# CliffKai/BridgeLang

Measured on AMD Instinct MI355X. Metric: action-seqs/sec (7-DoF, 224px) openvla-7b bf16, higher is better.
Workload: dtype bf16; 1 GPU; openvla-7b bf16 inference (BASELINE configs[1]): batch 16 synthetic 224px frames + 32-token prompts per GPU, predict_action = vision towers + projector + Llama prefill S=288 + 6 cached decode steps, greedy; 7 batches in flight: per step one batch is submitted (vision+prefill) while decode iteration g of the batch submitted g steps earlier, g = 1..6, runs as ONE merged 96-row pass over the weights ; batch_per_gpu=16, prompt_len=32, seq_len=288, replicas=1, hip_graph=True, pipeline_depth=7

## Files before the change

bridgelang_amd/_lib.py:

```python
from __future__ import annotations

import ctypes as C
import os
from pathlib import Path

_HERE = Path(__file__).resolve().parent
LIB_PATH = _HERE / "libbridgelang_hip.so"

BL_OK, BL_E_SHAPE, BL_E_ALIGN, BL_E_LAUNCH, BL_E_ARG = 0, -1, -2, -3, -4
_ERR = {BL_E_SHAPE: "BL_E_SHAPE (unsupported shape)", BL_E_ALIGN: "BL_E_ALIGN (alignment)",
        BL_E_LAUNCH: "BL_E_LAUNCH (HIP launch failed)", BL_E_ARG: "BL_E_ARG (null pointer / bad enum)"}

EPI_NONE, EPI_BIAS, EPI_BIAS_GELU, EPI_BIAS_RES, EPI_RES, EPI_SWIGLU, EPI_F32, EPI_F32_BF16R = range(8)
EPI_SWIGLU_KEEP, EPI_BIAS_GELU_KEEP, EPI_SWIGLU_BWD, EPI_GELU_BWD = range(8, 12)


class GemmDesc(C.Structure):
    _fields_ = [
        ("A", C.c_void_p), ("lda", C.c_int64),
        ("W", C.c_void_p), ("ldw", C.c_int64),
        ("C", C.c_void_p), ("ldc", C.c_int64),
        ("M", C.c_int32), ("N", C.c_int32), ("K", C.c_int32),
        ("epilogue", C.c_int32),
        ("bias", C.c_void_p),
# ... 14 lines not shown
    _fields_ = [("kind", C.c_int32), ("nblocks", C.c_int32), ("rows", C.c_int32), ("cols", C.c_int32), ("rows_pad", C.c_int32),
                ("bx_count", C.c_int32), ("ld", C.c_int64), ("kt_total", C.c_int64), ("kb_off", C.c_int64), ("n", C.c_int64),
                ("src", C.c_void_p), ("dst", C.c_void_p), ("scale", C.c_float), ("pad", C.c_int32)]


class AttnDesc(C.Structure):
    _fields_ = [
        ("q", C.c_void_p), ("q_bs", C.c_int64), ("q_hs", C.c_int64), ("q_rs", C.c_int64),
        ("k", C.c_void_p), ("k_bs", C.c_int64), ("k_hs", C.c_int64), ("k_rs", C.c_int64),
        ("v", C.c_void_p), ("v_bs", C.c_int64), ("v_hs", C.c_int64), ("v_rs", C.c_int64),
        ("o", C.c_void_p), ("o_bs", C.c_int64), ("o_hs", C.c_int64), ("o_rs", C.c_int64),
        ("key_mask", C.c_void_p), ("mask_bs", C.c_int64),
        ("B", C.c_int32), ("H", C.c_int32), ("Sq", C.c_int32), ("Skv", C.c_int32), ("head_dim", C.c_int32),
        ("causal", C.c_int32),
        ("scale", C.c_float),
    ]


_vp, _i32, _i64, _u32, _f32 = C.c_void_p, C.c_int32, C.c_int64, C.c_uint32, C.c_float

SIGNATURES = {
    "bl_abi_version": (C.c_int, []),
    "bl_build_arch": (C.c_char_p, []),
    "bl_fill_synth_bf16": (C.c_int, [_vp, _i64, _u32, _f32, _f32, _vp]),
    "bl_fill_synth_bf16_2d": (C.c_int, [_vp, _i64, _i64, _i64, _u32, _f32, _f32, _vp]),
    "bl_pack_weight_bf16": (C.c_int, [_vp, _i64, _i64, _i64, _vp, _vp]),
    "bl_gemm_fp8": (C.c_int, [C.POINTER(GemmDesc), _vp, _vp, _vp]),
    "bl_quantize_rows_fp8": (C.c_int, [_vp, _i64, _i32, _i32, _vp, _i64, _vp, _vp]),
    "bl_colamax_bf16": (C.c_int, [_vp, _i64, _i32, _i32, _vp, _vp]),
    "bl_transpose_quantize_fp8": (C.c_int, [_vp, _i64, _i32, _i32, _vp, _vp, _i64, _i32, _vp, _vp]),
    "bl_gemm_bf16": (C.c_int, [C.POINTER(GemmDesc), _vp]),
    "bl_gemm_skinny_bf16": (C.c_int, [C.POINTER(GemmDesc), _vp]),
    "bl_gemm_skinny_rows_bf16": (C.c_int, [C.POINTER(GemmDesc), _vp]),
    "bl_gemm_tn_bf16": (C.c_int, [C.POINTER(GemmDesc), _vp]),
    "bl_rmsnorm_skinny_bf16": (C.c_int, [_vp, _i64, _vp, _vp, _i64, _i32, _i32, _f32, _vp]),
    "bl_layernorm_bf16": (C.c_int, [_vp, _i64, _vp, _vp, _vp, _i64, _i32, _i32, _f32, _vp]),
    "bl_rmsnorm_bf16": (C.c_int, [_vp, _i64, _vp, _vp, _i64, _i32, _i32, _f32, _vp]),
    "bl_attention_bf16": (C.c_int, [C.POINTER(AttnDesc), _vp]),
    "bl_attention_rope_bf16": (C.c_int, [C.POINTER(AttnDesc), _vp, _vp, _i32, _vp, _vp, _i32, _vp]),
    "bl_attention_lse_bf16": (C.c_int, [C.POINTER(AttnDesc), _vp, _vp]),
    "bl_attention_backward_bf16": (C.c_int, [C.POINTER(AttnDesc), _vp, _vp, _vp, _vp, _vp, _vp, _vp]),
    "bl_attention_decode_bf16": (C.c_int, [C.POINTER(AttnDesc), _vp]),
    "bl_attention_decode_rope_bf16": (C.c_int, [C.POINTER(AttnDesc), _vp, _vp, _i32, _vp]),
    "bl_attention_decode_rope_pos_bf16": (C.c_int, [C.POINTER(AttnDesc), _vp, _vp, _i32, _vp, _vp]),
    "bl_attention_decode_rope_grouped_bf16": (C.c_int, [C.POINTER(AttnDesc), _vp, _vp, _i32, _vp, _vp, _vp, _vp]),
    "bl_rope_kvcache_bf16": (C.c_int, [_vp, _i32, _i32, _i32, _i32, _vp, _vp, _i32, _vp, _vp, _i32, _vp]),
    "bl_embed_splice_bf16": (C.c_int, [_vp, _i32, _i32, _vp, _i32, _i32, _vp, _vp]),
    "bl_argmax_f32": (C.c_int, [_vp, _i64, _i32, _i32, _vp, _vp]),
    "bl_cross_entropy_f32": (C.c_int, [_vp, _i64, _i32, _i32, _vp, _i64, _vp, _vp, _vp]),
    "bl_cross_entropy_backward_f32": (C.c_int, [_vp, _i64, _i32, _i32, _vp, _i64, _vp, _vp, _i64, _vp]),
    "bl_rmsnorm_backward_bf16": (C.c_int, [_vp, _i64, _vp, _vp, _i64, _vp, _i64, _vp, _i64, _vp, _vp, _i64, _i32, _i32, _f32, _vp]),
    "bl_layernorm_backward_bf16": (C.c_int, [_vp, _i64, _vp, _vp, _i64, _vp, _i64, _vp, _i64, _vp, _vp, _vp, _i64, _i32, _i32, _f32, _vp]),
    "bl_colsum_bf16": (C.c_int, [_vp, _i64, _i32, _i32, _vp, _vp, _i64, _vp]),
    "bl_swiglu_bf16": (C.c_int, [_vp, _i64, _vp, _i64, _i64, _i32, _vp]),
    "bl_swiglu_backward_bf16": (C.c_int, [_vp, _i64, _vp, _i64, _vp, _i64, _i64, _i32, _vp]),
    "bl_gelu_bf16": (C.c_int, [_vp, _i64, _vp, _i64, _i64, _i32, _vp]),
    "bl_gelu_backward_bf16": (C.c_int, [_vp, _i64, _vp, _i64, _vp, _i64, _i64, _i32, _vp]),
    "bl_rope_backward_bf16": (C.c_int, [_vp, _i64, _i32, _i32, _i32, _i32, _vp, _vp, _i32, _vp]),
    "bl_transpose_pad_bf16": (C.c_int, [_vp, _i64, _i32, _i32, _vp, _i64, _i32, _vp]),
    "bl_pack_weight_into_bf16": (C.c_int, [_vp, _i64, _i64, _i64, _vp, _i64, _i64, _vp]),
    "bl_transpose_pack_into_bf16": (C.c_int, [_vp, _i64, _i32, _i32, _vp, _i32, _i64, _i64, _vp]),
    "bl_transpose_pack_bf16": (C.c_int, [_vp, _i64, _i32, _i32, _vp, _i32, _vp]),
    "bl_sumsq_partial_f32": (C.c_int, [_vp, _i64, _vp, _i32, _vp]),
    "bl_clip_coef_f32": (C.c_int, [_vp, _i32, _f32, _vp, _vp]),
    "bl_adamw_f32": (C.c_int, [_vp, _vp, _vp, _vp, _vp, _i64, _f32, _f32, _f32, _f32, _f32, _i32, _vp, _vp]),
    "bl_rope_bf16": (C.c_int, [_vp, _i64, _i32, _i32, _i32, _i32, _vp, _vp, _i32, _vp]),
# ... 51 lines not shown
```

bridgelang_amd/csrc/gemm_bf16.hip:

```cpp
#include "gemm_common.h"
#include <stdlib.h>

namespace bl_gemm_bf16_impl {
using namespace blgemm;

constexpr int BK = 64;
constexpr int ROW_BYTES = 128;
constexpr int GROUP_M = 4;

__device__ __forceinline__ void lin_to_tile(const GemmArgs& p, int lin, int& tm, int& tn) {
  const int width = GROUP_M * p.tiles_n, grp = lin / width, first = grp * GROUP_M;
  const int gsz = min(p.tiles_m - first, GROUP_M), rem = lin - grp * width;
  tm = first + rem % gsz;
  tn = rem / gsz;
}

__device__ __forceinline__ void tile_coords(const GemmArgs& p, int& tm, int& tn) {
  const int nwg = gridDim.x;
  const int orig = blockIdx.x, xcd = orig & 7, q = nwg >> 3, r = nwg & 7;
  const int lin = (xcd < r ? xcd * (q + 1) : r * (q + 1) + (xcd - r) * q) + (orig >> 3);
  const int width = GROUP_M * p.tiles_n, grp = lin / width, first = grp * GROUP_M;
  const int gsz = min(p.tiles_m - first, GROUP_M), rem = lin - grp * width;
  tm = first + rem % gsz;
  tn = rem / gsz;
// ... 1121 lines not shown
  f32x4_t sum = {0.f, 0.f, 0.f, 0.f};
  for (int s = 0; s < p.splitk; ++s)
    sum += *(const f32x4_t*)(p.slab + (((long)(tile_local * p.splitk + s) * 32 + idx) * 512 + tid) * 4);
  epilogue_store4<EPI>(p, tm * 256 + wm * 128 + j * 16 + l15,
                       TN ? tn * 256 + (i >> 1) * 128 + wn * 32 + (i & 1) * 16 + lg * 4 : tn * 256 + wn * 64 + i * 16 + lg * 4, sum);
}

constexpr int CUS = 256;
constexpr int LDS128 = 2 * 256 * ROW_BYTES, LDS256 = 2 * 65536, LDS288 = 2 * 73728;
constexpr int ring8_lds_bytes(int bm, int bn) { return 4 * (bm + bn) * ROW_BYTES + 1024; }

template <typename Kernel>
bool lds_attr(Kernel* kernel, int bytes) {
  return hipFuncSetAttribute(reinterpret_cast<const void*>(kernel), hipFuncAttributeMaxDynamicSharedMemorySize, bytes) ==
         hipSuccess;
}

template <int MB, int NB>
constexpr int mid_lds_bytes() { return 3 * (64 * MB * ROW_BYTES + NB * 2048); }
template <int EPI, int MB, int NB, int SK = 0>
bool mid_attr() { return lds_attr(&gemm_mid_kernel<EPI, MB, NB, SK>, mid_lds_bytes<MB, NB>()); }

constexpr int RS_LDS_BYTES = 4 * 2 * 6 * 16 * ROW_BYTES;
template <int EPI, int NWV, int SK>
int launch_rs(const GemmArgs& p, hipStream_t s, int n_tiles) {
  static const int attr_rc = lds_attr(&gemm_rows_stream_kernel<EPI, NWV, SK>, RS_LDS_BYTES) ? BL_OK : BL_E_LAUNCH;
  if (attr_rc != BL_OK) return attr_rc;
  hipLaunchKernelGGL((gemm_rows_stream_kernel<EPI, NWV, SK>), dim3((n_tiles + NWV - 1) / NWV, 8 / SK), dim3(NWV * 64),
                     RS_LDS_BYTES, s, p, n_tiles);
  return BL_OK;
}

template <int EPI>
int launch_rows_sk(const GemmArgs& a, hipStream_t s) {
  static const int attr_rc = mid_attr<EPI, 2, 4, 8>() && mid_attr<EPI, 2, 4, 2>() ? BL_OK : BL_E_LAUNCH;
  if (attr_rc != BL_OK) return attr_rc;
  GemmArgs p = a;
  p.fold_ks = p.K / 256;
  const int n_tiles = p.N / 16;
  const char* e_on = getenv("BL_ROWS_STREAM");
  if (p.M <= 96 && p.fold_ks % 4 == 0 && n_tiles > 256 && (e_on ? atoi(e_on) : 1)) {
    const bool can_split = p.slab && p.slab_bytes >= 2L * p.M * p.N * 4;
    int rc;
    if ((n_tiles + 7) / 8 >= 200) {
      p.splitk = 1;
      rc = launch_rs<EPI, 8, 8>(p, s, n_tiles);
    } else if ((n_tiles + 5) / 6 >= 200 || !can_split) {
      p.splitk = 1;
      rc = launch_rs<EPI, 6, 8>(p, s, n_tiles);
    } else {
      p.splitk = 2;
      rc = launch_rs<BL_EPI_NONE, 8, 4>(p, s, n_tiles);
      const long work = (long)p.M * (p.N / 4);
      if (rc == BL_OK)
        hipLaunchKernelGGL((gemm_rows_tree_reduce_kernel<EPI>), dim3((int)min((work + 255) / 256, 2048L)), dim3(256), 0, s, p);
    }
    if (rc != BL_OK) return rc;
    BL_CHECK_LAUNCH();
    return BL_OK;
  }
  const int slabs64 = (p.N + 63) / 64;
  const bool split = slabs64 * 2 <= 256 && p.slab && p.slab_bytes >= 4L * p.M * p.N * 4;
  p.splitk = split ? 4 : 1;
  if (split) {
    hipLaunchKernelGGL((gemm_mid_kernel<EPI, 2, 4, 2>), dim3(slabs64, 4), dim3(256), (mid_lds_bytes<2, 4>()), s, p);
    const long work = (long)p.M * (p.N / 4);
    hipLaunchKernelGGL((gemm_rows_tree_reduce_kernel<EPI>), dim3((int)min((work + 255) / 256, 2048L)), dim3(256), 0, s, p);
  } else {
    hipLaunchKernelGGL((gemm_mid_kernel<EPI, 2, 4, 8>), dim3(slabs64), dim3(256), (mid_lds_bytes<2, 4>()), s, p);
  }
  BL_CHECK_LAUNCH();
  return BL_OK;
}

template <int EPI>
int set_lds_attr() {
  static const int rc = [] {
    const bool ok =
        lds_attr(&gemm256s_kernel<EPI>, LDS256) && lds_attr(&gemm288s_kernel<EPI>, LDS288) &&
        lds_attr(&gemm128_kernel<EPI>, LDS128) &&
        lds_attr(&gemm_ring8_kernel<EPI, 160, 128, 4>, ring8_lds_bytes(160, 128)) &&
        lds_attr(&gemm_ring8_kernel<EPI, 128, 128, 4>, ring8_lds_bytes(128, 128)) &&
        lds_attr(&gemm_ring8_kernel<EPI, 128, 64, 4>, ring8_lds_bytes(128, 64)) &&
        lds_attr(&gemm_ring8_kernel<EPI, 64, 64, 4>, ring8_lds_bytes(64, 64)) &&
        lds_attr(&gemm_mid2_kernel<EPI, 1>, 3 * (160 * ROW_BYTES + 4096)) &&
        lds_attr(&gemm_mid2_kernel<EPI, 4>, 3 * (160 * ROW_BYTES + 4 * 4096)) &&
        lds_attr(&gemm_mid2_kernel<EPI, 2, 2>, 2 * (160 * ROW_BYTES + 2 * 4096)) &&
        mid_attr<EPI, 2, 4>() && mid_attr<EPI, 4, 4>() && mid_attr<EPI, 5, 4>() && mid_attr<EPI, 2, 1>() &&
        mid_attr<EPI, 4, 1>() && mid_attr<EPI, 5, 1>();
    return ok ? BL_OK : BL_E_LAUNCH;
  }();
  return rc;
}

template <int EPI>
void launch_slab_reduce(const GemmArgs& p, hipStream_t s) {
  const long work = (long)p.M * (p.N / 4);
  hipLaunchKernelGGL((gemm128_splitk_reduce_kernel<EPI>), dim3((int)min((work + 255) / 256, 2048L)), dim3(256), 0, s, p);
}

template <int EPI, int MB>
void launch_mid(const GemmArgs& p, hipStream_t s, bool wide, dim3 grid) {
  if (wide) hipLaunchKernelGGL((gemm_mid_kernel<EPI, MB, 4>), grid, dim3(256), (mid_lds_bytes<MB, 4>()), s, p);
  else hipLaunchKernelGGL((gemm_mid_kernel<EPI, MB, 1>), grid, dim3(256), (mid_lds_bytes<MB, 1>()), s, p);
}
// ... 175 lines not shown
    case BL_EPI_NONE: return launch_gemm<BL_EPI_NONE>(a, s);
    case BL_EPI_BIAS: return launch_gemm<BL_EPI_BIAS>(a, s);
    case BL_EPI_BIAS_GELU: return launch_gemm<BL_EPI_BIAS_GELU>(a, s);
    case BL_EPI_BIAS_RES: return launch_gemm<BL_EPI_BIAS_RES>(a, s);
    case BL_EPI_RES: return launch_gemm<BL_EPI_RES>(a, s);
    case BL_EPI_SWIGLU: return launch_gemm<BL_EPI_SWIGLU>(a, s);
    case BL_EPI_F32: return launch_gemm<BL_EPI_F32>(a, s);
    case BL_EPI_F32_BF16R: return launch_gemm<BL_EPI_F32_BF16R>(a, s);
    case BL_EPI_SWIGLU_KEEP: return launch_gemm<BL_EPI_SWIGLU_KEEP>(a, s);
    case BL_EPI_BIAS_GELU_KEEP: return launch_gemm<BL_EPI_BIAS_GELU_KEEP>(a, s);
    case BL_EPI_SWIGLU_BWD: return launch_gemm<BL_EPI_SWIGLU_BWD>(a, s);
    case BL_EPI_GELU_BWD: return launch_gemm<BL_EPI_GELU_BWD>(a, s);
    default: return BL_E_ARG;
  }
}

extern "C" int bl_gemm_skinny_rows_bf16(const bl_gemm_desc* d, void* stream) {
  GemmArgs a;
  const int rc = fill_gemm_args(d, a);
  if (rc != BL_OK) return rc;
  if (d->M > 128 || (d->K % 256) || d->a_norm_weight) return BL_E_SHAPE;
  if (d->out_group) return BL_E_ARG;
  hipStream_t s = (hipStream_t)stream;
  switch (d->epilogue) {
    case BL_EPI_NONE: return launch_rows_sk<BL_EPI_NONE>(a, s);
    case BL_EPI_RES: return launch_rows_sk<BL_EPI_RES>(a, s);
    case BL_EPI_SWIGLU: return launch_rows_sk<BL_EPI_SWIGLU>(a, s);
    case BL_EPI_F32: return launch_rows_sk<BL_EPI_F32>(a, s);
    case BL_EPI_F32_BF16R: return launch_rows_sk<BL_EPI_F32_BF16R>(a, s);
    default: return BL_E_ARG;
  }
}

extern "C" int bl_gemm_tn_bf16(const bl_gemm_desc* d, void* stream) {
  if (!d || !d->A || !d->W || !d->C) return BL_E_ARG;
  if (d->epilogue != BL_EPI_F32 || d->out_group || d->a_norm_weight) return BL_E_ARG;
  if (d->M <= 0 || d->N <= 0 || d->K <= 0 || (d->M % 8) || (d->N % 8)) return BL_E_SHAPE;
  if ((d->lda % 8) || (d->ldw % 8) || (d->ldc % 4) || d->lda < d->M || d->ldw < d->N || d->ldc < d->N) return BL_E_ALIGN;
  if (!bl_aligned16(d->A) || !bl_aligned16(d->W) || (((uintptr_t)d->C) & 15)) return BL_E_ALIGN;
  if ((long)d->K * d->lda * 2 >= (1L << 31) || (long)d->K * d->ldw * 2 >= (1L << 31)) return BL_E_SHAPE;
  GemmArgs a = {};
  a.A = d->A; a.W = d->W; a.C = d->C;
  a.lda = d->lda; a.ldw = d->ldw; a.ldc = d->ldc;
  a.M = d->M; a.N = d->N; a.K = d->K;
  a.tail_base = -1;
  a.slab = (float*)d->workspace; a.slab_bytes = d->workspace_bytes; a.splitk = 1;
  return launch_gemm_tn(a, (hipStream_t)stream);
}
```

bridgelang_amd/csrc/gemm_common.h:

```cpp
#pragma once
#include "bl_common.h"

namespace blgemm {

struct GemmArgs {
  const uint16_t* A; const uint16_t* W; void* C;
  const uint16_t* bias; const uint16_t* scale; const uint16_t* res;
  long lda, ldw, ldc, ldres;
  int M, N, K;
  int res_row_mod, out_group, out_stride, out_offset;
  int tiles_m, tiles_n;
  const uint16_t* norm_w; float norm_eps;
  float* slab; long slab_bytes; int splitk;
  int tail_base;
  const float* qa; const float* qw;
  int fold_ks;
  uint16_t* C2; long ldc2;
  int ptiles;
};

__device__ __forceinline__ int out_row_of(const GemmArgs& p, int m) {
  if (p.out_group == 0) return m;
  const int g = m / p.out_group, r = m - g * p.out_group + p.out_offset;
  if (r < 0 || r >= p.out_stride) return -1;
  return g * p.out_stride + r;
}

template <int EPI>
__device__ __forceinline__ void epilogue_store4(const GemmArgs& p, int m, int n, f32x4_t acc) {
  if (m >= p.M || n >= p.N) return;
  const int orow = out_row_of(p, m);
  if (orow < 0) return;
  if constexpr (EPI == BL_EPI_F32 || EPI == BL_EPI_F32_BF16R) {
    float* c = (float*)p.C + (long)orow * p.ldc + n;
    if constexpr (EPI == BL_EPI_F32_BF16R) acc = (f32x4_t){rbf(acc[0]), rbf(acc[1]), rbf(acc[2]), rbf(acc[3])};
    *(f32x4_t*)c = acc;
    return;
  } else if constexpr (EPI == BL_EPI_SWIGLU_KEEP) {
    const float g0 = rbf(acc[0]), u0 = rbf(acc[1]), g1 = rbf(acc[2]), u1 = rbf(acc[3]);
    u32x2_t o; o[0] = pack2bf(g0, u0); o[1] = pack2bf(g1, u1);
    *(u32x2_t*)((uint16_t*)p.C + (long)orow * p.ldc + n) = o;
    *(uint32_t*)(p.C2 + (long)orow * p.ldc2 + (n >> 1)) = pack2bf(rbf(silu_f(g0)) * u0, rbf(silu_f(g1)) * u1);
    return;
  } else if constexpr (EPI == BL_EPI_SWIGLU_BWD) {
    float v[8], o[8];
    const u32x4_t q = *(const u32x4_t*)(p.res + (long)m * p.ldres + 2 * n);
#pragma unroll
    for (int i = 0; i < 4; ++i) { v[2 * i] = bflo(q[i]); v[2 * i + 1] = bfhi(q[i]); }
#pragma unroll
    for (int e = 0; e < 4; ++e) swiglu_bwd_pair(v[2 * e], v[2 * e + 1], rbf(acc[e]), o[2 * e], o[2 * e + 1]);
    u32x4_t w;
#pragma unroll
// ... 227 lines not shown
```

bridgelang_amd/csrc/gemm_skinny.hip:

```cpp
#include "gemm_common.h"

namespace bl_gemm_skinny_impl {
using namespace blgemm;

constexpr int NW = 8;

template <int KS>
__device__ __forceinline__ void load_x_fragments(const uint16_t* A, long lda, int M, int l15, long kbase,
                                                 bf16x8_t (&xf)[KS]) {
  const bool live = l15 < M;
  const uint16_t* xp = A + (long)(live ? l15 : M - 1) * lda + kbase;
#pragma unroll
  for (int s = 0; s < KS; ++s) {
    u32x4_t t = *(const u32x4_t*)(xp + s * 32);
    if (!live) t = (u32x4_t){0u, 0u, 0u, 0u};
    xf[s] = __builtin_bit_cast(bf16x8_t, t);
  }
}

template <int KS>
__device__ __forceinline__ void rmsnorm_fragments(const uint16_t* norm_w, float eps, int K, long kbase, int wave, int l15,
                                                  int lg, float (&nrm)[8][16], bf16x8_t (&xf)[KS]) {
  u32x4_t gw[KS];
  {
// ... 88 lines not shown
                          ((r[4][lane] + r[5][lane]) + (r[6][lane] + r[7][lane]));
      epilogue_store4<EPI>(p, l15, tile * 16 + lg * 4, sum);
    }
  }
#undef BL_LOAD_GROUP
}

template <int KS, int GS, int EPI>
int launch_ks(const GemmArgs& a, hipStream_t s) {
  const int n_tiles = a.N / 16;
  const int tpw = (n_tiles + 255) / 256;
  const int grid = (n_tiles + tpw - 1) / tpw;
  if (a.norm_w) hipLaunchKernelGGL((gemm_skinny_kernel<KS, GS, EPI, true>), dim3(grid), dim3(NW * 64), 0, s, a, n_tiles);
  else hipLaunchKernelGGL((gemm_skinny_kernel<KS, GS, EPI, false>), dim3(grid), dim3(NW * 64), 0, s, a, n_tiles);
  BL_CHECK_LAUNCH();
  return BL_OK;
}

template <int EPI>
int launch_skinny(const GemmArgs& a, hipStream_t s) {
  switch (a.K) {
    case 4096: return launch_ks<16, 8, EPI>(a, s);
    case 11008: return launch_ks<43, 8, EPI>(a, s);
    case 5120: return launch_ks<20, 5, EPI>(a, s);
    case 13824: return launch_ks<54, 9, EPI>(a, s);
    case 512: return launch_ks<2, 1, EPI>(a, s);
    case 1024: return launch_ks<4, 2, EPI>(a, s);
    case 1536: return launch_ks<6, 3, EPI>(a, s);
    default: return BL_E_SHAPE;
  }
}


template <int KS>
__global__ __launch_bounds__(NW * 64) void rmsnorm_skinny_kernel(const uint16_t* x, long ldx, const uint16_t* w,
                                                                 uint16_t* y, long ldy, int rows, int K, float eps) {
  __shared__ float nrm[NW][16];
  const int tid = threadIdx.x, lane = tid & 63, wave = tid >> 6;
  const int l15 = lane & 15, lg = lane >> 4;
  const long kbase = (long)wave * (KS * 32) + lg * 8;
  const int row0 = blockIdx.x * 16, m = min(16, rows - row0);
  bf16x8_t xf[KS];
  load_x_fragments<KS>(x + (long)row0 * ldx, ldx, m, l15, kbase, xf);
  rmsnorm_fragments<KS>(w, eps, K, kbase, wave, l15, lg, nrm, xf);
  if (l15 < m) {
    uint16_t* yp = y + (long)(row0 + l15) * ldy + kbase;
#pragma unroll
    for (int s = 0; s < KS; ++s) *(u32x4_t*)(yp + s * 32) = __builtin_bit_cast(u32x4_t, xf[s]);
  }
}

template <int KS>
int launch_norm_skinny(const uint16_t* x, long ldx, const uint16_t* w, uint16_t* y, long ldy, int rows, int K, float eps,
                       hipStream_t s) {
  hipLaunchKernelGGL((rmsnorm_skinny_kernel<KS>), dim3((rows + 15) / 16), dim3(NW * 64), 0, s, x, ldx, w, y, ldy, rows, K, eps);
  BL_CHECK_LAUNCH();
  return BL_OK;
}

}
using namespace bl_gemm_skinny_impl;

extern "C" int bl_gemm_skinny_bf16(const bl_gemm_desc* d, void* stream) {
  GemmArgs a;
  const int rc = fill_gemm_args(d, a);
  if (rc != BL_OK) return rc;
  if (d->M > 16) return BL_E_SHAPE;
  hipStream_t s = (hipStream_t)stream;
  switch (d->epilogue) {
    case BL_EPI_NONE: return launch_skinny<BL_EPI_NONE>(a, s);
    case BL_EPI_RES: return launch_skinny<BL_EPI_RES>(a, s);
    case BL_EPI_SWIGLU: return launch_skinny<BL_EPI_SWIGLU>(a, s);
    case BL_EPI_F32: return launch_skinny<BL_EPI_F32>(a, s);
    case BL_EPI_F32_BF16R: return launch_skinny<BL_EPI_F32_BF16R>(a, s);
    default: return BL_E_ARG;
  }
}

extern "C" int bl_rmsnorm_skinny_bf16(const bl_bf16* x, int64_t ldx, const bl_bf16* w, bl_bf16* y, int64_t ldy,
                                      int32_t rows, int32_t dim, float eps, void* stream) {
  if (!x || !w || !y) return BL_E_ARG;
  if (rows <= 0) return BL_E_SHAPE;
  if ((ldx % 8) || (ldy % 8) || ldx < dim || ldy < dim || !bl_aligned16(x) || !bl_aligned16(y) || !bl_aligned16(w))
    return BL_E_ALIGN;
  hipStream_t s = (hipStream_t)stream;
  switch (dim) {
    case 4096: return launch_norm_skinny<16>(x, ldx, w, y, ldy, rows, dim, eps, s);
    case 11008: return launch_norm_skinny<43>(x, ldx, w, y, ldy, rows, dim, eps, s);
    case 5120: return launch_norm_skinny<20>(x, ldx, w, y, ldy, rows, dim, eps, s);
    case 13824: return launch_norm_skinny<54>(x, ldx, w, y, ldy, rows, dim, eps, s);
    case 512: return launch_norm_skinny<2>(x, ldx, w, y, ldy, rows, dim, eps, s);
    case 1024: return launch_norm_skinny<4>(x, ldx, w, y, ldy, rows, dim, eps, s);
    case 1536: return launch_norm_skinny<6>(x, ldx, w, y, ldy, rows, dim, eps, s);
    default: return BL_E_SHAPE;
// ... 3 lines not shown
```

bridgelang_amd/ops.py:

```python
from __future__ import annotations

import functools
import math

import ctypes as C
from typing import Optional, Sequence, Tuple

import torch

from . import _lib
from ._lib import (AttnDesc, GemmDesc, EPI_BIAS, EPI_BIAS_GELU, EPI_BIAS_GELU_KEEP, EPI_BIAS_RES, EPI_F32, EPI_F32_BF16R, EPI_GELU_BWD,
                   EPI_NONE, EPI_SWIGLU_BWD, EPI_SWIGLU_KEEP,
                   EPI_RES, EPI_SWIGLU)

__all__ = ["Op", "gemm", "gemm_fp8", "quantize_rows_fp8", "quantize_weight_fp8", "pack_weight", "unpack_weight", "cross_entropy", "layernorm", "rmsnorm", "rmsnorm_skinny", "skinny_rows_supported", "attention", "attention_rope", "attention_decode", "attention_decode_rope", "attention_decode_rope_grouped", "skinny_supported", "rope_kvcache", "embed_splice",
           "argmax", "im2col_patch14", "preprocess_u8", "resample_coeffs", "resize_bicubic_u8", "resize_u8", "crop_resize_bilinear_u8", "write_prefix_tokens", "fill_synth", "run_all",
           "EPI_NONE", "EPI_BIAS", "EPI_BIAS_GELU", "EPI_BIAS_RES", "EPI_RES", "EPI_SWIGLU", "EPI_F32", "EPI_F32_BF16R",
           "EPI_SWIGLU_KEEP", "EPI_BIAS_GELU_KEEP", "EPI_SWIGLU_BWD", "EPI_GELU_BWD"]


def _stream() -> int:
    return torch.cuda.current_stream().cuda_stream


# ... 42 lines not shown
    lib = _lib.load()
    _bf16(w, "w")
    N, K = w.shape
    if out is None:
        out = torch.empty(N // 16, K // 32, 64, 8, dtype=torch.bfloat16, device=w.device)
    _lib.check(lib.bl_pack_weight_bf16(w.data_ptr(), _rows(w, "w"), N, K, _bf16(out, "out").data_ptr(), _stream()),
               "bl_pack_weight_bf16")
    return out


def unpack_weight(wp: torch.Tensor) -> torch.Tensor:
    nt, ks = wp.shape[0], wp.shape[1]
    return wp.view(nt, ks, 4, 16, 8).permute(0, 3, 1, 2, 4).reshape(nt * 16, ks * 32)


SKINNY_K = (512, 1024, 1536, 4096, 5120, 11008, 13824)
_SKINNY_EPI = (EPI_NONE, EPI_RES, EPI_SWIGLU, EPI_F32, EPI_F32_BF16R)


def skinny_supported(M: int, K: int, epilogue: int) -> bool:
    return M <= 16 and K in SKINNY_K and epilogue in _SKINNY_EPI


def skinny_rows_supported(M: int, K: int, epilogue: int) -> bool:
    return M <= 128 and K in SKINNY_K and epilogue in _SKINNY_EPI


def gemm(A: torch.Tensor, W: torch.Tensor, out: torch.Tensor, epilogue: int = EPI_NONE, *,
         bias: Optional[torch.Tensor] = None, scale: Optional[torch.Tensor] = None,
         res: Optional[torch.Tensor] = None, res_row_mod: int = 0,
         out_map: Optional[Tuple[int, int, int]] = None,
         skinny: Optional[bool] = None, algo_nk: Optional[Tuple[int, int]] = None,
         a_norm: Optional[Tuple[torch.Tensor, float]] = None, workspace: Optional[torch.Tensor] = None,
         skinny_rows: bool = False, out2: Optional[torch.Tensor] = None, run: bool = True) -> Op:
    lib = _lib.load()
    _bf16(A, "A"); _bf16(W, "W")
    if W.dim() != 4 or W.shape[2:] != (64, 8) or not W.is_contiguous():
        raise ValueError(f"gemm: W must be a packed weight [N/16, K/32, 64, 8] (ops.pack_weight), got {tuple(W.shape)}")
    M, K = A.shape
    N, Kw = W.shape[0] * 16, W.shape[1] * 32
    if Kw != K:
        raise ValueError(f"gemm: K mismatch A{tuple(A.shape)} W(packed) K={Kw}")
    want = torch.float32 if epilogue in (EPI_F32, EPI_F32_BF16R) else torch.bfloat16
    if out.dtype != want or not out.is_cuda:
        raise TypeError(f"gemm: out must be {want} on device")
    d = GemmDesc()
    d.A, d.lda = A.data_ptr(), _rows(A, "A")
    d.W, d.ldw = W.data_ptr(), K
    d.C, d.ldc = out.data_ptr(), _rows(out, "out")
    d.M, d.N, d.K, d.epilogue = M, N, K, epilogue
    keep = [A, W, out]
    if bias is not None:
        d.bias = _bf16(bias, "bias").data_ptr(); keep.append(bias)
    if scale is not None:
        d.scale = _bf16(scale, "scale").data_ptr(); keep.append(scale)
    if res is not None:
        d.res, d.ldres = _bf16(res, "res").data_ptr(), _rows(res, "res"); keep.append(res)
    d.res_row_mod = res_row_mod
    if epilogue in (EPI_SWIGLU_KEEP, EPI_BIAS_GELU_KEEP):
        if out2 is None:
            raise ValueError("gemm: the *_KEEP epilogues need out2")
        n2 = N // 2 if epilogue == EPI_SWIGLU_KEEP else N
        if out2.shape[1] < n2 or out2.shape[0] < M:
            raise ValueError(f"gemm: out2 {tuple(out2.shape)} too small for [{M}, {n2}]")
        d.C2, d.ldc2 = _bf16(out2, "out2").data_ptr(), _rows(out2, "out2"); keep.append(out2)
    elif out2 is not None:
        raise ValueError("gemm: out2 only with the *_KEEP epilogues")
    if epilogue in (EPI_SWIGLU_BWD, EPI_GELU_BWD) and (res is None or res.shape[0] < M or
                                                       res.shape[1] < (2 * N if epilogue == EPI_SWIGLU_BWD else N)):
        raise ValueError("gemm: the *_BWD epilogues read the saved pre-activation through res")
    if out_map is not None:
        d.out_group, d.out_stride, d.out_offset = out_map
    if workspace is not None:
        d.workspace, d.workspace_bytes = workspace.data_ptr(), workspace.numel() * workspace.element_size()
        keep.append(workspace)
    n_out = N // 2 if epilogue == EPI_SWIGLU else 2 * N if epilogue == EPI_SWIGLU_BWD else N
    if out.shape[1] < n_out:
        raise ValueError(f"gemm: out has {out.shape[1]} columns, needs {n_out}")
    if out_map is None and out.shape[0] < M:
        raise ValueError(f"gemm: out has {out.shape[0]} rows, needs {M}")
    use_skinny = skinny
    if use_skinny is None:
        use_skinny = skinny_supported(M, K, epilogue)
    if a_norm is not None:
        if not use_skinny:
            raise ValueError("gemm: a_norm (fused RMSNorm) needs the skinny kernel (M <= 16 and a supported K)")
        d.a_norm_weight, d.a_norm_eps = _bf16(a_norm[0], "a_norm weight").data_ptr(), float(a_norm[1])
        keep.append(a_norm[0])
    if skinny_rows:
        if not skinny_rows_supported(M, K, epilogue) or a_norm is not None or out_map is not None:
            raise ValueError(f"gemm: skinny_rows needs M <= 128, K in {SKINNY_K}, no a_norm / out_map (M={M}, K={K})")
        name = "bl_gemm_skinny_rows_bf16"
    else:
        name = "bl_gemm_skinny_bf16" if use_skinny else "bl_gemm_bf16"
    fn = getattr(lib, name)
    esz = 4 if epilogue in (EPI_F32, EPI_F32_BF16R) else 2
    op = Op(name, fn, (C.byref(d),), (d, *keep),
            flops=2.0 * M * (algo_nk[0] if algo_nk else N) * (algo_nk[1] if algo_nk else K),
            nbytes=2.0 * (M * K + N * K) + esz * M * n_out)
    if run:
        op.run()
    return op


FP8_MAX = 448.0


def quantize_weight_fp8(w: torch.Tensor) -> Tuple[torch.Tensor, torch.Tensor]:
    N, K = w.shape
    if N % 16 or K % 128:
        raise ValueError("quantize_weight_fp8: N % 16 == 0 and K % 128 == 0")
    wf = w.float()
    amax = wf.abs().amax(dim=1)
    scale = torch.where(amax > 0, amax / FP8_MAX, torch.ones_like(amax))
    q = (wf / scale[:, None]).to(torch.float8_e4m3fn)
    packed = pack_weight(q.view(torch.uint8).view(N, K // 2, 2).view(torch.bfloat16).reshape(N, K // 2).contiguous())
    return packed, scale.contiguous()


def quantize_rows_fp8(x: torch.Tensor, q: Optional[torch.Tensor] = None, scales: Optional[torch.Tensor] = None,
                      run: bool = True):
    lib = _lib.load()
    _bf16(x, "x")
    rows, cols = x.shape
    if q is None:
        q = torch.empty(rows, cols, dtype=torch.uint8, device=x.device)
    if scales is None:
        scales = torch.empty(rows, dtype=torch.float32, device=x.device)
    op = Op("bl_quantize_rows_fp8", lib.bl_quantize_rows_fp8,
            (x.data_ptr(), _rows(x, "x"), rows, cols, q.data_ptr(), q.stride(0), scales.data_ptr()), (x, q, scales),
            nbytes=3.0 * rows * cols)
    if run:
# ... 412 lines not shown
```

bridgelang_amd/pipeline.py:

```python
from __future__ import annotations

from typing import List, Optional, Sequence

import torch

from . import ops
from .engine import OpenVLAEngine
from .ops import EPI_F32_BF16R, EPI_NONE, EPI_RES, EPI_SWIGLU, Op
from .weights import VLAWeights


class TwoStagePipeline:
    def __init__(self, weights: VLAWeights, batch: int, prompt_len: int, n_new: int = 7):
        self.engines = [OpenVLAEngine(weights, batch, prompt_len, n_new) for _ in range(2)]
        self.device = weights.embed.device
        self._decode_stream = torch.cuda.Stream(device=self.device)
        self._graphs: List[Optional[torch.cuda.CUDAGraph]] = [None, None]
        self._tick = 0

    def _run_pair(self, k: int) -> None:
        e1, e2 = self.engines[k], self.engines[1 - k]
        main = torch.cuda.current_stream()
        self._decode_stream.wait_stream(main)
        with torch.cuda.stream(self._decode_stream):
# ... 36 lines not shown

    def __init__(self, weights: VLAWeights, batch: int, prompt_len: int, n_new: int = 7, split_vision: bool = False,
                 fp8: bool = False):
        if n_new < 2:
            raise ValueError("StaggeredDecodePipeline needs at least one decode iteration (n_new >= 2)")
        self.w, self.dims, self.B, self.n_new = weights, weights.dims, batch, n_new
        self.split_vision = split_vision
        self.lag = 1 if split_vision else 0
        self.slots = n_new + self.lag
        self.engines = [OpenVLAEngine(weights, batch, prompt_len, n_new, fp8=fp8) for _ in range(self.slots)]
        self.device = dev = weights.embed.device
        d = self.dims
        G = n_new - 1
        M = G * batch
        z = lambda *shape, dtype=torch.bfloat16: torch.zeros(*shape, dtype=dtype, device=dev)
        self.xd, self.hd, self.aod = z(M, d.llm_dim), z(M, d.llm_dim), z(M, d.llm_dim)
        self.qkvd, self.actd = z(M, 3 * d.llm_dim), z(M, d.llm_inter)
        self.logits = z(M, d.vocab, dtype=torch.float32)
        self.ws = torch.empty(4 * min(M, 128) * d.llm_dim * 4, dtype=torch.uint8, device=dev)
        self._decode_stream = torch.cuda.Stream(device=dev)
        self._vision_stream = torch.cuda.Stream(device=dev)
        self._main_stream = torch.cuda.Stream(device=dev)
        self.merged_ops: List[List[Op]] = [self._plan_merged(k) for k in range(self.slots)]
        self._graphs: List[Optional[torch.cuda.CUDAGraph]] = [None] * self.slots
        self._tick = 0

    def _plan_merged(self, k: int) -> List[Op]:
        d, w, B = self.dims, self.w, self.B
        D, H, hd = d.llm_dim, d.llm_heads, d.head_dim
        e0 = self.engines[0]
        fused = ops.skinny_supported(B, D, EPI_NONE) and hd == 128
        M = self.xd.shape[0]

        def gm(A, W, out, epi, res=None):
            if not ops.skinny_supported(B, A.shape[1], epi):
                return [ops.gemm(A, W, out, epi, res=res, skinny=False, run=False)]
            return [ops.gemm(A[r0:r0 + 128], W, out[r0:r0 + 128], epi, res=None if res is None else res[r0:r0 + 128],
                             skinny_rows=True, workspace=self.ws, run=False) for r0 in range(0, M, 128)]

        def norm(x, wn, out, fused_in_engine):
            return (ops.rmsnorm_skinny if fused_in_engine else ops.rmsnorm)(x, wn, out, d.rms_eps, run=False)

        groups = [(g, self.engines[(k - g - self.lag) % self.slots], slice((g - 1) * B, g * B)) for g in range(1, self.n_new)]
        plan = [ops.embed_splice(e.gen_ids[g - 1].view(B, 1), w.embed, self.xd[r].view(B, 1, D), 0, run=False)
                for g, e, r in groups]
        for l, lw in enumerate(w.layers):
            plan.append(norm(self.xd, lw.ln1, self.hd, fused))
            plan += gm(self.hd, lw.qkv_w, self.qkvd, EPI_NONE)
            grouped = fused and len(groups) <= 8
            if grouped:
                plan.append(ops.attention_decode_rope_grouped(
                    self.qkvd, [e.k_cache[l] for _, e, _ in groups], [e.v_cache[l] for _, e, _ in groups], self.aod,
                    e0.cos, e0.sin, B=B, H=H, head_dim=hd, pos=[e.S + g - 1 for g, e, _ in groups], run=False))
            for g, e, r in groups:
                pos = e.S + g - 1
                if grouped:
                    continue
                if fused:
                    plan.append(ops.attention_decode_rope(self.qkvd[r], e.k_cache[l], e.v_cache[l], self.aod[r], e0.cos, e0.sin,
                                                          B=B, H=H, head_dim=hd, pos=pos, run=False))
                else:
                    cs = (H * e.cache_len * hd, e.cache_len * hd, hd)
                    plan.append(ops.rope_kvcache(self.qkvd[r], e0.cos, e0.sin, e.k_cache[l], e.v_cache[l], B=B, S=1, H=H,
                                                 head_dim=hd, pos0=pos, run=False))
                    plan.append(ops.attention_decode(self.qkvd[r], e.k_cache[l], e.v_cache[l], self.aod[r], B=B, H=H,
                                                     Skv=pos + 1, head_dim=hd, q_strides=(3 * D, hd, 3 * D), k_strides=cs,
                                                     v_strides=cs, o_strides=(D, hd, D), run=False))
            plan += gm(self.aod, lw.o_w, self.xd, EPI_RES, res=self.xd)
            plan.append(norm(self.xd, lw.ln2, self.hd, fused))
            plan += gm(self.hd, lw.gu_w, self.actd, EPI_SWIGLU)
            plan += gm(self.actd, lw.down_w, self.xd, EPI_RES, res=self.xd)
        plan.append(norm(self.xd, w.norm, self.hd, ops.skinny_supported(B, D, EPI_F32_BF16R)))
        plan += gm(self.hd, w.lm_head, self.logits, EPI_F32_BF16R)
        plan += [ops.argmax(self.logits[r], e.gen_ids[g], run=False) for g, e, r in groups]
        return plan

    def _run_tick(self, k: int) -> None:
        e1 = self.engines[k]
        main = torch.cuda.current_stream()
        self._decode_stream.wait_stream(main)
        with torch.cuda.stream(self._decode_stream):
            ops.run_all(self.merged_ops[k])
        if self.split_vision:
            vs, ss = self._vision_stream, e1._side
            vs.wait_stream(main)
            ss.wait_stream(main)
            with torch.cuda.stream(ss):
                ops.run_all(e1.siglip_ops)
            with torch.cuda.stream(vs):
                ops.run_all(e1.dino_ops)
                vs.wait_stream(ss)
                ops.run_all(e1.projector_ops)
            ops.run_all(self.engines[(k - 1) % self.slots].prefill_ops)
            main.wait_stream(vs)
        else:
            e1.run_vision()
            ops.run_all(e1.projector_ops + e1.prefill_ops)
        main.wait_stream(self._decode_stream)

    def capture(self) -> None:
        for k in range(self.slots):
            self._run_tick(k)
        torch.cuda.synchronize()
        for k in range(self.slots):
            g = torch.cuda.CUDAGraph()
# ... 33 lines not shown
```

include/bridgelang_hip.h:

```cpp
#ifndef BRIDGELANG_HIP_H
#define BRIDGELANG_HIP_H

#include <stdint.h>

#ifdef __cplusplus
extern "C" {
#endif

typedef uint16_t bl_bf16;

#define BL_OK 0
#define BL_E_SHAPE (-1)
#define BL_E_ALIGN (-2)
#define BL_E_LAUNCH (-3)
#define BL_E_ARG (-4)

int bl_abi_version(void);
const char* bl_build_arch(void);

int bl_fill_synth_bf16(bl_bf16* dst, int64_t n, uint32_t seed, float mean, float scale, void* stream);
int bl_fill_synth_bf16_2d(bl_bf16* dst, int64_t rows, int64_t cols, int64_t ld, uint32_t seed, float mean,
                          float scale, void* stream);

int bl_pack_weight_bf16(const bl_bf16* src, int64_t ld, int64_t n, int64_t k, bl_bf16* dst, void* stream);
// ... 7 lines not shown
  BL_EPI_SWIGLU = 5,
  BL_EPI_F32 = 6,
  BL_EPI_F32_BF16R = 7,
  BL_EPI_SWIGLU_KEEP = 8,
  BL_EPI_BIAS_GELU_KEEP = 9,
  BL_EPI_SWIGLU_BWD = 10,
  BL_EPI_GELU_BWD = 11
};

typedef struct bl_gemm_desc {
  const bl_bf16* A;  int64_t lda;
  const bl_bf16* W;  int64_t ldw;
  void* C;           int64_t ldc;
  int32_t M, N, K;
  int32_t epilogue;
  const bl_bf16* bias;
  const bl_bf16* scale;
  const bl_bf16* res; int64_t ldres;
  int32_t res_row_mod;
  int32_t out_group, out_stride, out_offset;
  const bl_bf16* a_norm_weight;
  float a_norm_eps;
  void* workspace;
  int64_t workspace_bytes;
  bl_bf16* C2;
  int64_t ldc2;
} bl_gemm_desc;

int bl_gemm_bf16(const bl_gemm_desc* d, void* stream);

int bl_gemm_skinny_bf16(const bl_gemm_desc* d, void* stream);

int bl_gemm_skinny_rows_bf16(const bl_gemm_desc* d, void* stream);

int bl_gemm_tn_bf16(const bl_gemm_desc* d, void* stream);

int bl_rmsnorm_skinny_bf16(const bl_bf16* x, int64_t ldx, const bl_bf16* w, bl_bf16* y, int64_t ldy, int32_t rows,
                           int32_t dim, float eps, void* stream);

int bl_gemm_fp8(const bl_gemm_desc* d, const float* scale_a, const float* scale_w, void* stream);
int bl_quantize_rows_fp8(const bl_bf16* x, int64_t ldx, int32_t rows, int32_t cols, uint8_t* q, int64_t ldq, float* scales,
                         void* stream);
int bl_colamax_bf16(const bl_bf16* x, int64_t ldx, int32_t rows, int32_t cols, float* amax, void* stream);
int bl_transpose_quantize_fp8(const bl_bf16* x, int64_t ldx, int32_t rows, int32_t cols, const float* amax, uint8_t* q,
                              int64_t ldq, int32_t packed, float* scales, void* stream);

int bl_layernorm_bf16(const bl_bf16* x, int64_t ldx, const bl_bf16* w, const bl_bf16* b, bl_bf16* y, int64_t ldy,
                      int32_t rows, int32_t dim, float eps, void* stream);
int bl_rmsnorm_bf16(const bl_bf16* x, int64_t ldx, const bl_bf16* w, bl_bf16* y, int64_t ldy, int32_t rows,
                    int32_t dim, float eps, void* stream);

typedef struct bl_attn_desc {
  const bl_bf16* q; int64_t q_bs, q_hs, q_rs;
  const bl_bf16* k; int64_t k_bs, k_hs, k_rs;
  const bl_bf16* v; int64_t v_bs, v_hs, v_rs;
  bl_bf16* o;       int64_t o_bs, o_hs, o_rs;
  const uint8_t* key_mask; int64_t mask_bs;
  int32_t B, H, Sq, Skv, head_dim;
  int32_t causal;
  float scale;
} bl_attn_desc;
int bl_attention_bf16(const bl_attn_desc* d, void* stream);
int bl_attention_rope_bf16(const bl_attn_desc* d, const bl_bf16* cos_tab, const bl_bf16* sin_tab, int32_t pos0, bl_bf16* k_cache,
                           bl_bf16* v_cache, int32_t cache_len, void* stream);
int bl_attention_lse_bf16(const bl_attn_desc* d, float* lse, void* stream);
int bl_attention_backward_bf16(const bl_attn_desc* d, const bl_bf16* dout, const float* lse, float* delta, bl_bf16* dq,
// ... 97 lines not shown
```

Before: 279.2 action-seqs/s.

## Fuse following RMSNorm into split-K reduce of residual skinny-row GEMMs

Adds a split-K finish kernel that sums the partial slabs, applies the residual add, writes the output, and computes the next RMSNorm from LDS-staged rows. The decode plan then fuses ln2 after o_proj and the next layer's ln1 (or the final norm) after down_proj into that finish step. Where the shape is unsupported it falls back to a separate norm. This removes one norm launch and one activation reread per fused GEMM. The trade-off is that the finish kernel uses fewer, LDS-heavy workgroups (4 rows each), which may parallelise worse than the tree-reduce it replaces. It also changes the default rows per workgroup of the standalone skinny norm from 16 to 4.

Result: no change. 278.6 action-seqs/s, median of 2 (-0.2%).

```diff
diff --git a/bridgelang_amd/_lib.py b/bridgelang_amd/_lib.py
--- a/bridgelang_amd/_lib.py
+++ b/bridgelang_amd/_lib.py
@@ -70,6 +70,7 @@
     "bl_gemm_bf16": (C.c_int, [C.POINTER(GemmDesc), _vp]),
     "bl_gemm_skinny_bf16": (C.c_int, [C.POINTER(GemmDesc), _vp]),
     "bl_gemm_skinny_rows_bf16": (C.c_int, [C.POINTER(GemmDesc), _vp]),
+    "bl_gemm_skinny_rows_norm_bf16": (C.c_int, [C.POINTER(GemmDesc), _vp, _f32, _vp, _i64, _vp]),
     "bl_gemm_tn_bf16": (C.c_int, [C.POINTER(GemmDesc), _vp]),
     "bl_rmsnorm_skinny_bf16": (C.c_int, [_vp, _i64, _vp, _vp, _i64, _i32, _i32, _f32, _vp]),
     "bl_layernorm_bf16": (C.c_int, [_vp, _i64, _vp, _vp, _vp, _i64, _i32, _i32, _f32, _vp]),
diff --git a/bridgelang_amd/csrc/gemm_bf16.hip b/bridgelang_amd/csrc/gemm_bf16.hip
--- a/bridgelang_amd/csrc/gemm_bf16.hip
+++ b/bridgelang_amd/csrc/gemm_bf16.hip
@@ -1177,11 +1177,25 @@
 }
 
 template <int EPI>
-int launch_rows_sk(const GemmArgs& a, hipStream_t s) {
+int launch_rows_sk(const GemmArgs& a, hipStream_t s, const OutNorm* on = nullptr) {
   static const int attr_rc = mid_attr<EPI, 2, 4, 8>() && mid_attr<EPI, 2, 4, 2>() ? BL_OK : BL_E_LAUNCH;
   if (attr_rc != BL_OK) return attr_rc;
   GemmArgs p = a;
   p.fold_ks = p.K / 256;
+  bool normed = false;
+  auto finish = [&](const GemmArgs& q) -> int {
+    if (on) {
+      const int rc = launch_rows_finish_norm(q, *on, s);
+      if (rc != BL_E_SHAPE) { normed = true; return rc; }
+    }
+    const long work = (long)q.M * (q.N / 4);
+    hipLaunchKernelGGL((gemm_rows_tree_reduce_kernel<EPI>), dim3((int)min((work + 255) / 256, 2048L)), dim3(256), 0, s, q);
+    return BL_OK;
+  };
+  auto norm_owed = [&]() -> int {
+    if (!on || normed) return BL_OK;
+    return bl_rmsnorm_skinny_bf16((const bl_bf16*)p.C, p.ldc, on->w, on->y, on->ldy, p.M, p.N, on->eps, s);
+  };
   const int n_tiles = p.N / 16;
   const char* e_on = getenv("BL_ROWS_STREAM");
   if (p.M <= 96 && p.fold_ks % 4 == 0 && n_tiles > 256 && (e_on ? atoi(e_on) : 1)) {
@@ -1196,26 +1210,24 @@
     } else {
       p.splitk = 2;
       rc = launch_rs<BL_EPI_NONE, 8, 4>(p, s, n_tiles);
-      const long work = (long)p.M * (p.N / 4);
-      if (rc == BL_OK)
-        hipLaunchKernelGGL((gemm_rows_tree_reduce_kernel<EPI>), dim3((int)min((work + 255) / 256, 2048L)), dim3(256), 0, s, p);
+      if (rc == BL_OK) rc = finish(p);
     }
     if (rc != BL_OK) return rc;
     BL_CHECK_LAUNCH();
-    return BL_OK;
+    return norm_owed();
   }
   const int slabs64 = (p.N + 63) / 64;
   const bool split = slabs64 * 2 <= 256 && p.slab && p.slab_bytes >= 4L * p.M * p.N * 4;
   p.splitk = split ? 4 : 1;
   if (split) {
     hipLaunchKernelGGL((gemm_mid_kernel<EPI, 2, 4, 2>), dim3(slabs64, 4), dim3(256), (mid_lds_bytes<2, 4>()), s, p);
-    const long work = (long)p.M * (p.N / 4);
-    hipLaunchKernelGGL((gemm_rows_tree_reduce_kernel<EPI>), dim3((int)min((work + 255) / 256, 2048L)), dim3(256), 0, s, p);
+    const int rc = finish(p);
+    if (rc != BL_OK) return rc;
   } else {
     hipLaunchKernelGGL((gemm_mid_kernel<EPI, 2, 4, 8>), dim3(slabs64), dim3(256), (mid_lds_bytes<2, 4>()), s, p);
   }
   BL_CHECK_LAUNCH();
-  return BL_OK;
+  return norm_owed();
 }
 
 template <int EPI>
@@ -1457,6 +1469,25 @@
   }
 }
 
+extern "C" int bl_gemm_skinny_rows_norm_bf16(const bl_gemm_desc* d, const bl_bf16* norm_w, float norm_eps, bl_bf16* y,
+                                             int64_t ldy, void* stream) {
+  GemmArgs a;
+  const int rc = fill_gemm_args(d, a);
+  if (rc != BL_OK) return rc;
+  if (!norm_w || !y) return BL_E_ARG;
+  if (d->M > 128 || (d->K % 256) || d->a_norm_weight) return BL_E_SHAPE;
+  if (d->out_group || d->epilogue != BL_EPI_RES) return BL_E_ARG;
+  switch (d->N) {
+    case 512: case 1024: case 1536: case 4096: case 5120: case 11008: case 13824: break;
+    default: return BL_E_SHAPE;
+  }
+  if ((d->ldc % 8) || (d->ldres % 8) || (ldy % 8) || d->ldc < d->N || d->ldres < d->N || ldy < d->N ||
+      !bl_aligned16(d->res) || !bl_aligned16(norm_w) || !bl_aligned16(y) || (d->workspace && !bl_aligned16(d->workspace)))
+    return BL_E_ALIGN;
+  const OutNorm on = {norm_w, norm_eps, y, (long)ldy};
+  return launch_rows_sk<BL_EPI_RES>(a, (hipStream_t)stream, &on);
+}
+
 extern "C" int bl_gemm_tn_bf16(const bl_gemm_desc* d, void* stream) {
   if (!d || !d->A || !d->W || !d->C) return BL_E_ARG;
   if (d->epilogue != BL_EPI_F32 || d->out_group || d->a_norm_weight) return BL_E_ARG;
diff --git a/bridgelang_amd/csrc/gemm_common.h b/bridgelang_amd/csrc/gemm_common.h
--- a/bridgelang_amd/csrc/gemm_common.h
+++ b/bridgelang_amd/csrc/gemm_common.h
@@ -18,6 +18,12 @@
   uint16_t* C2; long ldc2;
   int ptiles;
 };
+
+struct OutNorm {
+  const uint16_t* w; float eps;
+  uint16_t* y; long ldy;
+};
+int launch_rows_finish_norm(const GemmArgs& p, const OutNorm& on, hipStream_t s);
 
 __device__ __forceinline__ int out_row_of(const GemmArgs& p, int m) {
   if (p.out_group == 0) return m;
diff --git a/bridgelang_amd/csrc/gemm_skinny.hip b/bridgelang_amd/csrc/gemm_skinny.hip
--- a/bridgelang_amd/csrc/gemm_skinny.hip
+++ b/bridgelang_amd/csrc/gemm_skinny.hip
@@ -144,14 +144,20 @@
 }
 
 
-template <int KS>
+#ifndef BL_NORM_ROWS
+#define BL_NORM_ROWS 4
+#endif
+constexpr int NORM_ROWS = BL_NORM_ROWS;
+static_assert(NORM_ROWS == 1 || NORM_ROWS == 2 || NORM_ROWS == 4 || NORM_ROWS == 16, "rows per workgroup: 1, 2, 4 or 16");
+
+template <int KS, int R>
 __global__ __launch_bounds__(NW * 64) void rmsnorm_skinny_kernel(const uint16_t* x, long ldx, const uint16_t* w,
                                                                  uint16_t* y, long ldy, int rows, int K, float eps) {
   __shared__ float nrm[NW][16];
   const int tid = threadIdx.x, lane = tid & 63, wave = tid >> 6;
   const int l15 = lane & 15, lg = lane >> 4;
   const long kbase = (long)wave * (KS * 32) + lg * 8;
-  const int row0 = blockIdx.x * 16, m = min(16, rows - row0);
+  const int row0 = blockIdx.x * R, m = min(R, rows - row0);
   bf16x8_t xf[KS];
   load_x_fragments<KS>(x + (long)row0 * ldx, ldx, m, l15, kbase, xf);
   rmsnorm_fragments<KS>(w, eps, K, kbase, wave, l15, lg, nrm, xf);
@@ -165,13 +171,103 @@
 template <int KS>
 int launch_norm_skinny(const uint16_t* x, long ldx, const uint16_t* w, uint16_t* y, long ldy, int rows, int K, float eps,
                        hipStream_t s) {
-  hipLaunchKernelGGL((rmsnorm_skinny_kernel<KS>), dim3((rows + 15) / 16), dim3(NW * 64), 0, s, x, ldx, w, y, ldy, rows, K, eps);
+  hipLaunchKernelGGL((rmsnorm_skinny_kernel<KS, NORM_ROWS>), dim3((rows + NORM_ROWS - 1) / NORM_ROWS), dim3(NW * 64), 0, s,
+                     x, ldx, w, y, ldy, rows, K, eps);
   BL_CHECK_LAUNCH();
   return BL_OK;
 }
 
+#ifndef BL_FINISH_ROWS
+#define BL_FINISH_ROWS 4
+#endif
+constexpr int FINISH_ROWS = BL_FINISH_ROWS;
+
+template <int KS, int R, int S>
+__global__ __launch_bounds__(NW * 64) void rows_finish_norm_kernel(GemmArgs p, OutNorm on) {
+  constexpr int CPR = KS * 32;
+  constexpr int ITER = (R * CPR + NW * 64 - 1) / (NW * 64);
+  static_assert(R * CPR * 16 <= 65536, "the staged rows must fit static LDS");
+  __shared__ u32x4_t stage[R * CPR];
+  __shared__ float nrm[NW][16];
+  const int tid = threadIdx.x, lane = tid & 63, wave = tid >> 6;
+  const int l15 = lane & 15, lg = lane >> 4;
+  const long kbase = (long)wave * (KS * 32) + lg * 8;
+  const int row0 = blockIdx.x * R, m = min(R, p.M - row0);
+  const long stride = (long)p.M * p.N;
+#pragma unroll
+  for (int it = 0; it < ITER; ++it) {
+    const int idx = it * (NW * 64) + tid;
+    if (idx < m * CPR) {
+      const int row = row0 + idx / CPR, col = (idx % CPR) * 8;
+      const float* q = p.slab + (long)row * p.N + col;
+      f32x4_t v[S][2];
+#pragma unroll
+      for (int s2 = 0; s2 < S; ++s2) {
+        v[s2][0] = *(const f32x4_t*)(q + s2 * stride);
+        v[s2][1] = *(const f32x4_t*)(q + s2 * stride + 4);
+      }
+      const int rrow = p.res_row_mod ? (row % p.res_row_mod) : row;
+      const u32x4_t r = *(const u32x4_t*)(p.res + (long)rrow * p.ldres + col);
+#pragma unroll
+      for (int w = 1; w < S; w *= 2)
+#pragma unroll
+        for (int s2 = 0; s2 < S; s2 += 2 * w) {
+          v[s2][0] = v[s2][0] + v[s2 + w][0];
+          v[s2][1] = v[s2][1] + v[s2 + w][1];
+        }
+      u32x4_t o;
+#pragma unroll
+      for (int h = 0; h < 2; ++h) {
+        float e[4] = {v[0][h][0], v[0][h][1], v[0][h][2], v[0][h][3]};
+#pragma unroll
+        for (int i = 0; i < 4; ++i) e[i] = rbf(e[i]);
+        e[0] += bflo(r[2 * h]); e[1] += bfhi(r[2 * h]); e[2] += bflo(r[2 * h + 1]); e[3] += bfhi(r[2 * h + 1]);
+        o[2 * h] = pack2bf(e[0], e[1]); o[2 * h + 1] = pack2bf(e[2], e[3]);
+      }
+      *(u32x4_t*)((uint16_t*)p.C + (long)row * p.ldc + col) = o;
+      stage[idx] = o;
+    }
+  }
+  __syncthreads();
+  const bool live = l15 < m;
+  bf16x8_t xf[KS];
+#pragma unroll
+  for (int s = 0; s < KS; ++s) {
+    u32x4_t t = {0u, 0u, 0u, 0u};
+    if (live) t = stage[l15 * CPR + wave * (KS * 4) + s * 4 + lg];
+    xf[s] = __builtin_bit_cast(bf16x8_t, t);
+  }
+  rmsnorm_fragments<KS>(on.w, on.eps, p.N, kbase, wave, l15, lg, nrm, xf);
+  if (live) {
+    uint16_t* yp = on.y + (long)(row0 + l15) * on.ldy + kbase;
+#pragma unroll
+    for (int s = 0; s < KS; ++s) *(u32x4_t*)(yp + s * 32) = __builtin_bit_cast(u32x4_t, xf[s]);
+  }
+}
+
+template <int KS>
+int launch_finish_ks(const GemmArgs& p, const OutNorm& on, hipStream_t s) {
+  const dim3 grid((p.M + FINISH_ROWS - 1) / FINISH_ROWS), block(NW * 64);
+  if (p.splitk == 2) hipLaunchKernelGGL((rows_finish_norm_kernel<KS, FINISH_ROWS, 2>), grid, block, 0, s, p, on);
+  else if (p.splitk == 4) hipLaunchKernelGGL((rows_finish_norm_kernel<KS, FINISH_ROWS, 4>), grid, block, 0, s, p, on);
+  else return BL_E_ARG;
+  BL_CHECK_LAUNCH();
+  return BL_OK;
+}
+
 }
 using namespace bl_gemm_skinny_impl;
+
+int blgemm::launch_rows_finish_norm(const GemmArgs& p, const OutNorm& on, hipStream_t s) {
+  switch (p.N) {
+    case 4096: return launch_finish_ks<16>(p, on, s);
+    case 5120: return launch_finish_ks<20>(p, on, s);
+    case 512: return launch_finish_ks<2>(p, on, s);
+    case 1024: return launch_finish_ks<4>(p, on, s);
+    case 1536: return launch_finish_ks<6>(p, on, s);
+    default: return BL_E_SHAPE;
+  }
+}
 
 extern "C" int bl_gemm_skinny_bf16(const bl_gemm_desc* d, void* stream) {
   GemmArgs a;
diff --git a/bridgelang_amd/ops.py b/bridgelang_amd/ops.py
--- a/bridgelang_amd/ops.py
+++ b/bridgelang_amd/ops.py
@@ -98,7 +98,8 @@
          out_map: Optional[Tuple[int, int, int]] = None,
          skinny: Optional[bool] = None, algo_nk: Optional[Tuple[int, int]] = None,
          a_norm: Optional[Tuple[torch.Tensor, float]] = None, workspace: Optional[torch.Tensor] = None,
-         skinny_rows: bool = False, out2: Optional[torch.Tensor] = None, run: bool = True) -> Op:
+         skinny_rows: bool = False, out2: Optional[torch.Tensor] = None,
+         out_norm: Optional[Tuple[torch.Tensor, float, torch.Tensor]] = None, run: bool = True) -> Op:
     lib = _lib.load()
     _bf16(A, "A"); _bf16(W, "W")
     if W.dim() != 4 or W.shape[2:] != (64, 8) or not W.is_contiguous():
@@ -159,11 +160,22 @@
         name = "bl_gemm_skinny_rows_bf16"
     else:
         name = "bl_gemm_skinny_bf16" if use_skinny else "bl_gemm_bf16"
+    args, norm_bytes = (C.byref(d),), 0.0
+    if out_norm is not None:
+        wn, eps, y = out_norm
+        if not skinny_rows or epilogue != EPI_RES or N not in SKINNY_K:
+            raise ValueError(f"gemm: out_norm needs skinny_rows, EPI_RES and N in {SKINNY_K} (N={N})")
+        if y.shape[0] < M or y.shape[1] < N:
+            raise ValueError(f"gemm: out_norm y {tuple(y.shape)} too small for [{M}, {N}]")
+        name = "bl_gemm_skinny_rows_norm_bf16"
+        args += (_bf16(wn, "out_norm weight").data_ptr(), float(eps), _bf16(y, "out_norm y").data_ptr(), _rows(y, "out_norm y"))
+        keep += [wn, y]
+        norm_bytes = 2.0 * M * N
     fn = getattr(lib, name)
     esz = 4 if epilogue in (EPI_F32, EPI_F32_BF16R) else 2
-    op = Op(name, fn, (C.byref(d),), (d, *keep),
+    op = Op(name, fn, args, (d, *keep),
             flops=2.0 * M * (algo_nk[0] if algo_nk else N) * (algo_nk[1] if algo_nk else K),
-            nbytes=2.0 * (M * K + N * K) + esz * M * n_out)
+            nbytes=2.0 * (M * K + N * K) + esz * M * n_out + norm_bytes)
     if run:
         op.run()
     return op
diff --git a/bridgelang_amd/pipeline.py b/bridgelang_amd/pipeline.py
--- a/bridgelang_amd/pipeline.py
+++ b/bridgelang_amd/pipeline.py
@@ -92,20 +92,30 @@
         fused = ops.skinny_supported(B, D, EPI_NONE) and hd == 128
         M = self.xd.shape[0]
 
-        def gm(A, W, out, epi, res=None):
-            if not ops.skinny_supported(B, A.shape[1], epi):
-                return [ops.gemm(A, W, out, epi, res=res, skinny=False, run=False)]
-            return [ops.gemm(A[r0:r0 + 128], W, out[r0:r0 + 128], epi, res=None if res is None else res[r0:r0 + 128],
-                             skinny_rows=True, workspace=self.ws, run=False) for r0 in range(0, M, 128)]
-
         def norm(x, wn, out, fused_in_engine):
             return (ops.rmsnorm_skinny if fused_in_engine else ops.rmsnorm)(x, wn, out, d.rms_eps, run=False)
+
+        def gm(A, W, out, epi, res=None, then_norm=None):
+            rows = ops.skinny_supported(B, A.shape[1], epi)
+            joint = rows and then_norm is not None and then_norm[1] and out.shape[1] in ops.SKINNY_K
+            if not rows:
+                plan = [ops.gemm(A, W, out, epi, res=res, skinny=False, run=False)]
+            else:
+                plan = [ops.gemm(A[r0:r0 + 128], W, out[r0:r0 + 128], epi, res=None if res is None else res[r0:r0 + 128],
+                                 skinny_rows=True, workspace=self.ws, run=False,
+                                 out_norm=(then_norm[0], d.rms_eps, self.hd[r0:r0 + 128]) if joint else None)
+                        for r0 in range(0, M, 128)]
+            if then_norm is not None and not joint:
+                plan.append(norm(out, then_norm[0], self.hd, then_norm[1]))
+            return plan
 
         groups = [(g, self.engines[(k - g - self.lag) % self.slots], slice((g - 1) * B, g * B)) for g in range(1, self.n_new)]
         plan = [ops.embed_splice(e.gen_ids[g - 1].view(B, 1), w.embed, self.xd[r].view(B, 1, D), 0, run=False)
                 for g, e, r in groups]
+        head_norm_fused = ops.skinny_supported(B, D, EPI_F32_BF16R)
+        plan.append(norm(self.xd, w.layers[0].ln1, self.hd, fused))
         for l, lw in enumerate(w.layers):
-            plan.append(norm(self.xd, lw.ln1, self.hd, fused))
+            after_down = (w.layers[l + 1].ln1, fused) if l + 1 < len(w.layers) else (w.norm, head_norm_fused)
             plan += gm(self.hd, lw.qkv_w, self.qkvd, EPI_NONE)
             grouped = fused and len(groups) <= 8
             if grouped:
@@ -126,11 +136,9 @@
                     plan.append(ops.attention_decode(self.qkvd[r], e.k_cache[l], e.v_cache[l], self.aod[r], B=B, H=H,
                                                      Skv=pos + 1, head_dim=hd, q_strides=(3 * D, hd, 3 * D), k_strides=cs,
                                                      v_strides=cs, o_strides=(D, hd, D), run=False))
-            plan += gm(self.aod, lw.o_w, self.xd, EPI_RES, res=self.xd)
-            plan.append(norm(self.xd, lw.ln2, self.hd, fused))
+            plan += gm(self.aod, lw.o_w, self.xd, EPI_RES, res=self.xd, then_norm=(lw.ln2, fused))
             plan += gm(self.hd, lw.gu_w, self.actd, EPI_SWIGLU)
-            plan += gm(self.actd, lw.down_w, self.xd, EPI_RES, res=self.xd)
-        plan.append(norm(self.xd, w.norm, self.hd, ops.skinny_supported(B, D, EPI_F32_BF16R)))
+            plan += gm(self.actd, lw.down_w, self.xd, EPI_RES, res=self.xd, then_norm=after_down)
         plan += gm(self.hd, w.lm_head, self.logits, EPI_F32_BF16R)
         plan += [ops.argmax(self.logits[r], e.gen_ids[g], run=False) for g, e, r in groups]
         return plan
diff --git a/include/bridgelang_hip.h b/include/bridgelang_hip.h
--- a/include/bridgelang_hip.h
+++ b/include/bridgelang_hip.h
@@ -63,6 +63,9 @@
 int bl_gemm_skinny_bf16(const bl_gemm_desc* d, void* stream);
 
 int bl_gemm_skinny_rows_bf16(const bl_gemm_desc* d, void* stream);
+
+int bl_gemm_skinny_rows_norm_bf16(const bl_gemm_desc* d, const bl_bf16* norm_w, float norm_eps, bl_bf16* y, int64_t ldy,
+                                  void* stream);
 
 int bl_gemm_tn_bf16(const bl_gemm_desc* d, void* stream);
 
```
